# alipbcs/ZetaRay

Hardware: NVIDIA H100
Metric: Mpaths/s (1spp ReSTIR PT, 1080p) (higher is better)
Workload: dtype f32

## Files before the change

zetaray_b200/csrc/rdi.cu:

```cuda
#include "zr_pixel.cuh"
#include "zr_planes.h"
#include "zr_schedule.h"

#include "zr_rdi.cuh"

namespace zr
{
namespace
{
#ifndef ZR_RDI_THREADS
#define ZR_RDI_THREADS 512
#endif
    __global__ void ZR_LB(ZR_RDI_THREADS) k_di_temporal(SceneDev sc, FrameView f, DIParams prm, zr_rdi_reservoir* __restrict__ resCurr,
        const zr_rdi_reservoir* __restrict__ resPrev, uint2* __restrict__ target, float4* __restrict__ finalImg, uint32_t dispX, uint32_t dispY,
        const uint32_t* __restrict__ order)
    {
        const zr_frame_constants& fc = f.fc;
        uint2 sg = make_uint2(0, 0);
        const uint32_t groupFlat = order[blockIdx.x] * (ZR_RDI_THREADS / 64) + (threadIdx.x >> 6);
        const uint32_t tInGroup = threadIdx.x & 63;
        uint2 px = make_uint2(0xffffffffu, 0xffffffffu);
        if (groupFlat < dispX * dispY)
            px = SwizzleThreadGroup(groupFlat, 0, tInGroup & 7, tInGroup >> 3, 8, 8, dispX, 16, 4, 16 * dispY, sg);
        const long long t0 = clock64();
        bool act = !(px.x >= f.W || px.y >= f.H || px.y < prm.rowBegin || px.y >= prm.rowEnd);
        const uint32_t x = px.x, y = px.y;
        const size_t idx = act ? (size_t)y * f.W + x : 0;
        if (act)
        {
            const GFlags flags = FlagsAt(f.core, f.W, x, y);
            if (flags.invalid)
            {
                finalImg[idx] = f4(0, 0, 0, 0);
                act = false;
            }
            else if (flags.emissive && !prm.spatial)
            {
                WriteEmissive(fc, f, finalImg, idx);
                act = false;
            }
        }
        Pixel p;
        p.surface = BSDF::ShadingData::InitEmpty();
        p.pos = f3(0); p.normal = f3(0); p.roughness = 0;
        RNG rng_thread; rng_thread.State = 0;
        int numBsdfSamples = 0;
        if (act)
        {
            p = LoadPixel(f, sc, f.core, f.coat, x, y, false, x, y);
            rng_thread = RNG::Init(x, y, fc.FrameNum);
            numBsdfSamples = (!p.surface.GlossSpecular() && p.roughness < 0.3f) ? 2 : 1;
        }
        RNG rng_group = RNG::Init(groupFlat % dispX, groupFlat / dispX, fc.FrameNum);
        const uint32_t sampleSetIdx = rng_group.UniformUintBounded_Faster(sc.numSampleSets);
        Reservoir r = RIS_InitialCandidates_Sync(act, sc, p.pos, p.normal, p.roughness, p.surface, sampleSetIdx, numBsdfSamples, rng_thread);
        if (prm.temporal)
        {
            float2 motionVec = f2(0, 0);
            TemporalCandidate tc; tc.valid = false; tc.px = tc.py = 0; tc.pos = tc.normal = f3(0);
            tc.surface = BSDF::ShadingData::InitEmpty();
            ZR_PHASE();
            if (act)
            {
                motionVec = unpack_snorm16x2(__ldg(&f.me[idx].x));
                const float2 currUV = f2((float)x + 0.5f, (float)y + 0.5f) / f2((float)f.W, (float)f.H);
                const float2 prevUV = currUV - motionVec;
                tc = FindTemporalCandidate(f, sc, p.pos, p.normal, p.roughness, p.surface, prevUV);
            }
            TemporalResample1_Sync(act && tc.valid, sc, p.pos, p.normal, p.surface, tc, resPrev, f.W, r, rng_thread);
            if (act && prm.spatial)
            {
                const bool disoccluded = !tc.valid && (dot(motionVec, motionVec) > 0);
                r.target = disoccluded ? -r.target : r.target;
                WriteTarget(target, idx, r.target);
                r.target = Math::Sanitize(r.target);
            }
        }
        AccountCost(prm.costMap, f.W, f.H, px.x, px.y, t0);
        if (!act)
            return;
        if (prm.temporal || prm.reset)
        {
            zr_rdi_reservoir rec;
            r.Write(rec, prm.M_max);
            StoreRdi(&resCurr[idx], rec);
        }
        if (!prm.spatial || !prm.temporal)
            WriteFinal(fc, finalImg, idx, r.target * r.W);
    }

    __global__ void ZR_LB(ZR_RDI_THREADS) k_di_spatial(SceneDev sc, FrameView f, DIParams prm, const zr_rdi_reservoir* __restrict__ resCurr,
        const uint2* __restrict__ target, float4* __restrict__ finalImg, uint32_t dispX, uint32_t dispY,
        const uint32_t* __restrict__ order)
    {
        const zr_frame_constants& fc = f.fc;
        uint2 sg = make_uint2(0, 0);
        const uint32_t groupFlat = order[blockIdx.x] * (ZR_RDI_THREADS / 64) + (threadIdx.x >> 6);
        const uint32_t tInGroup = threadIdx.x & 63;
        uint2 px = make_uint2(0xffffffffu, 0xffffffffu);
        if (groupFlat < dispX * dispY)
            px = SwizzleThreadGroup(groupFlat, 0, tInGroup & 7, tInGroup >> 3, 8, 8, dispX, 16, 4, 16 * dispY, sg);
        const long long t0 = clock64();
        bool active = px.x < f.W && px.y < f.H && px.y >= prm.rowBegin && px.y < prm.rowEnd;
        const int x = (int)px.x, y = (int)px.y;
        const size_t idx = active ? (size_t)y * f.W + x : 0;
        if (active)
        {
            const GFlags flags = FlagsAt(f.core, f.W, x, y);
            if (flags.invalid) active = false;
            else if (flags.emissive)
            {
                WriteEmissive(fc, f, finalImg, idx);
                active = false;
            }
        }
        Pixel p;
        p.surface = BSDF::ShadingData::InitEmpty();
        p.pos = f3(0); p.normal = f3(0); p.roughness = 0; p.z = 0;
        Reservoir r = Reservoir::Init();
        bool disoccluded = false;
        if (active)
        {
            p = LoadPixel(f, sc, f.core, f.coat, x, y, false, x, y);
            zr_rdi_reservoir rec;
            LoadRdi(&resCurr[idx], rec);
            r = Reservoir::Load(rec);
            if (r.lightIdx != UINT32_MAX_)
            {
                const zr_emissive_tri& tri = sc.emissives[r.lightIdx];
                r.lightID = tri.ID;
                const float3 vtx0 = Light::Vtx0(tri);
                const float3 vtx1 = Light::DecodeEmissiveTriV1(tri);
                const float3 vtx2 = Light::DecodeEmissiveTriV2(tri);
                r.lightPos = (1.0f - r.bary.x - r.bary.y) * vtx0 + r.bary.x * vtx1 + r.bary.y * vtx2;
                r.lightNormal = cross(vtx1 - vtx0, vtx2 - vtx0);
                r.lightNormal = dot(r.lightNormal, r.lightNormal) == 0 ? r.lightNormal : normalize(r.lightNormal);
                r.doubleSided = Light::IsDoubleSided(tri);
                r.target = LoadTarget(target, idx);
                disoccluded = r.target.x < 0 || r.target.y < 0 || r.target.z < 0;
                r.target = abs3(r.target);
            }
        }
        const uint32_t waveDisoccluded = __popc(__ballot_sync(0xffffffffu, active && disoccluded));
        RNG rng_group = RNG::Init(groupFlat % dispX, groupFlat / dispX, fc.FrameNum);
        rng_group.UniformUintBounded_Faster(sc.numSampleSets);
        const bool extra = !prm.stochasticSpatial || (rng_group.Uniform() < 0.6f);
        if (prm.extraDisocclusion)
            disoccluded = disoccluded && (waveDisoccluded > 3);
        int numSamples = extra ? 2 : 1;
        numSamples = !disoccluded ? numSamples : 4;
        RNG rng = RNG::Init((uint32_t)x, (uint32_t)y, fc.FrameNum);
        const float u0 = rng.Uniform();
        const int offset = (int)rng.UniformUintBounded_Faster(8);
        const float theta = u0 * TWO_PI;
        float sinTheta, cosTheta;
        zr_sincosf(theta, &sinTheta, &cosTheta);
        PairwiseMIS pairwiseMIS = PairwiseMIS::Init((uint32_t)numSamples, r);
        float3 samplePos[4]; int spx[4], spy[4]; uint32_t k = 0;
        ZR_PHASE();
        for (int i = 0; i < 4; i++)
        {
            if (!(active && i < numSamples)) continue;
            const float2 sampleUV = f2(c_disk32[((offset + i) & 31) * 2], c_disk32[((offset + i) & 31) * 2 + 1]);
            float2 rotated;
            rotated.x = dot(sampleUV, f2(cosTheta, -sinTheta));
            rotated.y = dot(sampleUV, f2(sinTheta, cosTheta));
            rotated = rotated * 16.0f;
            const float fx = fmaxf(rintf((float)x + rotated.x), 0.0f), fy = fmaxf(rintf((float)y + rotated.y), 0.0f);
            if (fx >= (float)f.W || fy >= (float)f.H) continue;
            const int qx = (int)fx, qy = (int)fy;
            float rough_i;
            const GFlags flags_i = FlagsAt(f.core, f.W, qx, qy, &rough_i);
            if (flags_i.invalid || flags_i.emissive) continue;
            const Pixel pi = LoadPixel(f, sc, f.core, f.coat, qx, qy, false, qx, qy);
            bool valid = PlaneHeuristicDI(pi.pos, p.normal, p.pos, p.z);
            valid = valid && (fabsf(rough_i - p.roughness) < 0.15f);
            if (!valid) continue;
            samplePos[k] = pi.pos; spx[k] = qx; spy[k] = qy;
            k++;
        }
        pairwiseMIS.k = k;
        for (uint32_t i = 0; i < 4; i++)
        {
            const bool go = active && (i < k);
            if (!__syncthreads_or(go))
                break;
            Pixel pi;
            pi.normal = f3(0);
            BSDF::ShadingData surface_i = BSDF::ShadingData::InitEmpty();
            Reservoir r_spatial = Reservoir::Init();
            float3 pos_i = f3(0);
            if (go)
            {
                pi = LoadPixel(f, sc, f.core, f.coat, spx[i], spy[i], false, spx[i], spy[i]);
                const uint4 c = ld128(&f.core[(size_t)spy[i] * f.W + spx[i]]);
                const float3 bc = f3((float)(c.z & 0xff) / 255.0f, (float)((c.z >> 8) & 0xff) / 255.0f, (float)((c.z >> 16) & 0xff) / 255.0f);
                const float bw = pi.flags.subsurface ? (float)(c.z >> 24) / 255.0f : 0.0f;
                pos_i = samplePos[i];
                const float3 wo_i = normalize(pi.origin - pos_i);
                surface_i = BSDF::ShadingData::Init(pi.normal, wo_i, pi.flags.metallic, pi.roughness, bc, BSDF::ETA_AIR,
                    pi.eta_next, pi.flags.transmissive, 0.0f, to_half(bw), pi.surface.coat_weight, pi.surface.coat_color,
                    pi.coatRoughness, pi.coatIor, sc.rho);
                zr_rdi_reservoir recN;
                LoadRdi(&resCurr[(size_t)spy[i] * f.W + spx[i]], recN);
                r_spatial = Reservoir::Load(recN);
            }
            pairwiseMIS.Stream_Sync(go, sc, r, p.pos, p.normal, p.surface, r_spatial, pos_i, pi.normal, surface_i, rng);
        }
        AccountCost(prm.costMap, f.W, f.H, px.x, px.y, t0);
        if (!active)
            return;
        pairwiseMIS.End(r, rng);
        const Reservoir rs = pairwiseMIS.r_s;
        WriteFinal(fc, finalImg, idx, rs.target * rs.W);
    }
}
}

struct zr_direct_pass
{
    uint32_t width = 0, height = 0;
    struct Sized
    {
        zr::Planes planes{ "zr_direct_pass" };
        zr_rdi_reservoir* d_res[2] = { nullptr, nullptr };
        uint2* d_target = nullptr;
        float4* d_final = nullptr;
    } sz;
    int currTemporalIdx = 0;
    bool isTemporalReservoirValid = false;
    bool resetTemporalTextures = true;
    bool patternLoaded = false;
    zr_direct_params params = Defaults();
    zr::LightingStrip strip{ "zr_direct_pass" };

    static zr_direct_params Defaults()
    {
        zr_direct_params p{};
        p.temporal_resample = 1; p.spatial_resample = 1; p.stochastic_spatial = 1; p.extra_disocclusion_sampling = 1;
        p.M_max = 20; p.alpha_min = 0.05f * 0.05f;
        return p;
    }
    zr_status Setup() { return ZR_OK; }
    zr_status OnWindowResized(uint32_t w, uint32_t h)
    {
        const size_t n = (size_t)w * h;
        Sized next;
        for (int i = 0; i < 2; i++) ZR_TRY(next.planes.Alloc(next.d_res[i], n));
        ZR_TRY(next.planes.Alloc(next.d_target, n));
        ZR_TRY(next.planes.Alloc(next.d_final, n));
        ZR_TRY(next.planes.Clear());
        sz = std::move(next);
        width = w; height = h;
        strip.ForgetSize();
        ResetFlags();
        return ZR_OK;
    }
    void ResetFlags() { currTemporalIdx = 0; isTemporalReservoirValid = false; resetTemporalTextures = true; }
    zr_status ResetTemporal()
    {
        ZR_TRY(sz.planes.Clear());
        ResetFlags();
        return ZR_OK;
    }
    zr_status LoadPattern()
    {
        if (patternLoaded) return ZR_OK;
        float pat[64];
        zr_status st = zr::read_asset("zr_direct_pass", "disk32.bin", pat, sizeof(pat));
        if (st != ZR_OK) return st;
        ZR_CUDA(cudaMemcpyToSymbol(zr::c_disk32, pat, 256));
        patternLoaded = true;
        return ZR_OK;
    }
    zr_status Render(const zr_frame_inputs* in, cudaStream_t stream)
    {
        using namespace zr;
        FrameView f;
        zr_status st = LightingFrame("zr_direct_pass", in, width, height, f);
        if (st != ZR_OK) return st;
        st = LoadPattern();
        if (st != ZR_OK) return st;
        const bool doTemporal = isTemporalReservoirValid && params.temporal_resample;
        const bool doSpatial = doTemporal && params.spatial_resample;
        if (doTemporal && (!in->prev.d_core || !in->prev.d_coat))
        {
            set_error("zr_direct_pass_render: temporal reuse needs the previous G-buffer");
            return ZR_ERR_INVALID_ARG;
        }
        DIParams prm{ doTemporal, doSpatial, params.stochastic_spatial, params.extra_disocclusion_sampling, params.M_max,
            params.alpha_min, resetTemporalTextures, strip.rowBegin, strip.ClampedRowEnd(height), strip.d_costMap };
        const uint32_t dispX = (width + 7) / 8, dispY = (height + 7) / 8;
        const int cur = currTemporalIdx;
        st = strip.Schedule(width, height, 8, 8, ZR_RDI_THREADS / 64);
        if (st != ZR_OK) return st;
        const BlockSchedule& sched = strip.sched;
        ZR_PROF("k_di_temporal", stream);
        k_di_temporal<<<sched.count, ZR_RDI_THREADS, 0, stream>>>(in->scene->dev, f, prm, sz.d_res[cur], sz.d_res[1 - cur], sz.d_target, sz.d_final, dispX, dispY, sched.d_order);
        ZR_LAUNCH_CHECK();
        strip.Exchange(sz.d_res[cur], width, height, 32u, stream);
        if (doSpatial)
        {
            ZR_PROF("k_di_spatial", stream);
            k_di_spatial<<<sched.count, ZR_RDI_THREADS, 0, stream>>>(in->scene->dev, f, prm, sz.d_res[cur], sz.d_target, sz.d_final, dispX, dispY, sched.d_order);
            ZR_LAUNCH_CHECK();
        }
        isTemporalReservoirValid = true;
        currTemporalIdx = 1 - cur;
        resetTemporalTextures = false;
        return ZR_OK;
    }
};

extern "C"
{
    zr_status zr_direct_pass_create(uint32_t width, uint32_t height, zr_direct_pass** out) { return zr::CreatePass("zr_direct_pass", width, height, out); }
    zr_status zr_direct_pass_resize(zr_direct_pass* p, uint32_t width, uint32_t height) { return zr::ResizePass("zr_direct_pass", p, width, height); }
    zr_status zr_direct_pass_reset_temporal(zr_direct_pass* p) { return zr::ResetPass(p); }
    zr_status zr_direct_pass_default_params(zr_direct_params* out) { return zr::DefaultParams<zr_direct_pass>(out); }
    zr_status zr_direct_pass_set_params(zr_direct_pass* p, const zr_direct_params* params)
    {
        if (!p || !params) return ZR_ERR_INVALID_ARG;
        if (params->M_max == 0 || params->M_max > 31) { zr::set_error("zr_direct_pass_set_params: M_max must be in 1..31 (5-bit field)"); return ZR_ERR_INVALID_ARG; }
        p->params = *params;
        return ZR_OK;
    }
    zr_status zr_direct_pass_render(zr_direct_pass* p, const zr_frame_inputs* in, void* stream)
    {
        if (!p) return ZR_ERR_INVALID_ARG;
        return p->Render(in, (cudaStream_t)stream);
    }
    zr_status zr_direct_pass_set_rows(zr_direct_pass* p, uint32_t y0, uint32_t y1) { return p ? p->strip.SetRows(y0, y1, p->height) : ZR_ERR_INVALID_ARG; }
    zr_status zr_direct_pass_set_halo_exchange(zr_direct_pass* p, zr_halo_exchange_fn fn, void* user) { return p ? p->strip.SetHaloExchange(fn, user) : ZR_ERR_INVALID_ARG; }
    zr_status zr_direct_pass_set_schedule_costs(zr_direct_pass* p, const double* h_tile_cost, uint32_t tiles_x, uint32_t tiles_y)
    {
        return p ? p->strip.SetScheduleCosts(h_tile_cost, tiles_x, tiles_y, p->width, p->height) : ZR_ERR_INVALID_ARG;
    }
    zr_status zr_direct_pass_set_cost_map(zr_direct_pass* p, void* d_cycles) { return p ? p->strip.SetCostMap(d_cycles) : ZR_ERR_INVALID_ARG; }
    zr_status zr_direct_pass_get_output(zr_direct_pass* p, zr_direct_output id, zr_image2d* out)
    {
        if (!p || !out) return ZR_ERR_INVALID_ARG;
        const uint32_t w = p->width, h = p->height;
        switch (id)
        {
        case ZR_DIRECT_FINAL: *out = zr_image2d{ p->sz.d_final, w, h, w * 16u, 16u }; break;
        case ZR_DIRECT_RESERVOIR_CURR: *out = zr_image2d{ p->sz.d_res[1 - p->currTemporalIdx], w, h, w * 32u, 32u }; break;
        case ZR_DIRECT_TARGET: *out = zr_image2d{ p->sz.d_target, w, h, w * 8u, 8u }; break;
        default: zr::set_error("zr_direct_pass_get_output: unknown output id"); return ZR_ERR_INVALID_ARG;
        }
        return ZR_OK;
    }
    zr_status zr_direct_pass_describe_io(zr_direct_pass* p, zr_resource_use* uses, int* n)
    {
        if (!p || !uses || !n) return ZR_ERR_INVALID_ARG;
        uses[0] = zr_resource_use{ ZR_RES_GBUFFER_CURR, 0 };
        uses[1] = zr_resource_use{ ZR_RES_GBUFFER_PREV, 0 };
        uses[2] = zr_resource_use{ ZR_RES_SCENE_BVH, 0 };
        uses[3] = zr_resource_use{ ZR_RES_ALIAS_TABLE, 0 };
        uses[4] = zr_resource_use{ ZR_RES_DI_FINAL, 1 };
        *n = 5;
        return ZR_OK;
    }
    void zr_direct_pass_destroy(zr_direct_pass* p) { delete p; }
}
```

zetaray_b200/csrc/zr_rdi.cuh:

```cuda
#pragma once
#include "zr_pixel.cuh"

namespace zr
{
namespace
{
    struct DIParams
    {
        uint32_t temporal, spatial, stochasticSpatial, extraDisocclusion, M_max; float alpha_min; uint32_t reset;
        uint32_t rowBegin, rowEnd;
        unsigned long long* costMap;
    };

    __constant__ float c_disk32[64];

struct Reservoir
{
    float w_sum, W; float3 le; uint32_t lightIdx; float2 bary; uint32_t M;
    float3 target; uint32_t lightID; float3 lightPos, lightNormal; bool doubleSided;

    static ZR_D Reservoir Init()
    {
        Reservoir r;
        r.le = f3(0); r.M = 0; r.w_sum = 0; r.W = 0; r.lightIdx = UINT32_MAX_; r.bary = f2(0, 0);
        r.target = f3(0); r.lightID = UINT32_MAX_; r.lightPos = f3(0); r.lightNormal = f3(0); r.doubleSided = false;
        return r;
    }
    ZR_D bool Update(float weight, float3 le_, uint32_t lightIdx_, float2 bary_, RNG& rng)
    {
        if (weight != weight) return false;
        M += 1;
        if (weight == 0) return false;
        w_sum += weight;
        if (rng.Uniform() < (weight / w_sum))
        {
            le = le_; lightIdx = lightIdx_; bary = bary_;
            return true;
        }
        return false;
    }
    static ZR_D Reservoir Load(const zr_rdi_reservoir& s)
    {
        Reservoir r = Init();
        r.le = f3(half_lo(s.le_rg), half_hi(s.le_rg), half_lo(s.le_b_meta));
        r.M = (s.le_b_meta >> 16) & 0x1f;
        r.w_sum = s.w_sum; r.W = s.W;
        r.lightIdx = s.lightIdx;
        r.bary = Math::DecodeUNorm2(s.bary);
        return r;
    }
    ZR_D void Write(zr_rdi_reservoir& s, uint32_t M_max) const
    {
        uint32_t M_capped = M < M_max ? M : M_max;
        s.bary = Math::EncodeUNorm2(bary);
        s.le_rg = pack_half2(le.x, le.y);
        s.le_b_meta = (uint32_t)zr_f32_to_f16(le.z) | (M_capped << 16);
        s.lightIdx = lightIdx;
        s.w_sum = w_sum; s.W = W;
        s.pad[0] = 0; s.pad[1] = 0;
    }
};

ZR_D void WriteTarget(uint2* target, size_t idx, float3 t)
{
    t = Math::Sanitize(t);
    target[idx] = make_uint2(pack_half2(t.x, t.y), pack_half2(t.z, 0.0f));
}
ZR_D float3 LoadTarget(const uint2* target, size_t idx)
{
    uint2 p = target[idx];
    return f3(half_lo(p.x), half_hi(p.x), half_lo(p.y));
}

struct BSDFHitInfo { uint32_t emissiveTriIdx; float2 bary; float3 lightPos; float t; bool hit; };

ZR_D BSDFHitInfo FindClosestHitDI(const SceneDev& sc, float3 pos, float3 normal, float3 wi, bool transmissive)
{
    BSDFHitInfo ret;
    ret.hit = false; ret.emissiveTriIdx = UINT32_MAX_; ret.bary = f2(0, 0); ret.lightPos = f3(0); ret.t = 0;
    float ndotwi = dot(normal, wi);
    if (ndotwi == 0) return ret;
    bool wiBackface = ndotwi < 0;
    if (wiBackface)
    {
        if (transmissive) normal = -normal;
        else return ret;
    }
    const float3 adjustedOrigin = RTU::OffsetRayRTG(pos, normal);
    RayHit h = TraceClosest(sc, adjustedOrigin, wi, wiBackface ? 3e-4f : 0.0f, FLT_MAX_);
    if (h.hit)
    {
        const uint32_t meshIdx = __ldg(&sc.triMesh[h.tri]);
        const uint32_t baseEmissive = __ldg(&sc.instances[meshIdx].BaseEmissiveTriOffset);
        if (baseEmissive == UINT32_MAX_)
            return ret;
        ret.emissiveTriIdx = baseEmissive + (h.tri - __ldg(&sc.meshFirstTri[meshIdx]));
        ret.bary = h.bary;
        ret.lightPos = mad(h.t, wi, adjustedOrigin);
        ret.t = h.t;
        ret.hit = true;
    }
    return ret;
}

struct EmissiveData
{
    float3 wi; float t; uint32_t ID; float3 lightPos, lightNormal; bool doubleSided;
    static ZR_D EmissiveData Init(const SceneDev& sc, uint32_t lightIdx, float2 bary)
    {
        EmissiveData ret;
        const zr_emissive_tri& tri = sc.emissives[lightIdx];
        ret.ID = tri.ID;
        const float3 vtx0 = Light::Vtx0(tri);
        const float3 vtx1 = Light::DecodeEmissiveTriV1(tri);
        const float3 vtx2 = Light::DecodeEmissiveTriV2(tri);
        ret.lightPos = (1.0f - bary.x - bary.y) * vtx0 + bary.x * vtx1 + bary.y * vtx2;
        ret.lightNormal = cross(vtx1 - vtx0, vtx2 - vtx0);
        ret.lightNormal = dot(ret.lightNormal, ret.lightNormal) == 0 ? ret.lightNormal : normalize(ret.lightNormal);
        ret.doubleSided = Light::IsDoubleSided(tri);
        ret.wi = f3(0); ret.t = 0;
        return ret;
    }
    ZR_D void SetSurfacePos(float3 pos)
    {
        wi = lightPos - pos;
        t = dot(wi, wi) == 0 ? 0 : length(wi);
        wi = t == 0 ? f3(0) : wi / t;
        lightNormal = doubleSided && dot(-wi, lightNormal) < 0 ? -lightNormal : lightNormal;
    }
    ZR_D float dWdA() const
    {
        float cosThetaPrime = saturate(dot(lightNormal, -wi));
        return t == 0 ? 0 : cosThetaPrime / (t * t);
    }
};

#define ZR_PHASE() __syncthreads()
ZR_D Reservoir RIS_InitialCandidates_Sync(bool act, const SceneDev& sc, float3 pos, float3 normal, float roughness, BSDF::ShadingData surface,
    uint32_t sampleSetIdx, int numBsdfSamples, RNG& rng)
{
    Reservoir r = Reservoir::Init();
    const bool specular = surface.GlossSpecular() && (surface.metallic || surface.specTr) && (!surface.Coated() || surface.CoatSpecular());
    const int numLightSamples = !specular ? 3 : 0;
    for (int s_b = 0; s_b < 2; s_b++)
    {
        const bool go = act && (s_b < numBsdfSamples);
        BSDF::BSDFSample bsdfSample = BSDF::BSDFSample::Init();
        ZR_PHASE();
        if (go)
            bsdfSample = BSDF::SampleBSDF_NoDiffuse(normal, surface, rng);
        ZR_PHASE();
        BSDFHitInfo hitInfo;
        hitInfo.hit = false;
        if (go)
            hitInfo = FindClosestHitDI(sc, pos, normal, bsdfSample.wi, surface.Transmissive());
        ZR_PHASE();
        if (go)
        {
            float3 wi = bsdfSample.wi;
            float pdf_w = bsdfSample.pdf;
            float w_b = 0;
            float3 le = f3(0), lightNormal = f3(0), target = f3(0);
            uint32_t emissiveID = UINT32_MAX_;
            bool doubleSided = false;
            if (hitInfo.hit)
            {
                const zr_emissive_tri& emissive = sc.emissives[hitInfo.emissiveTriIdx];
                le = Light::Le_EmissiveTriangle(emissive);
                const float3 vtx0 = Light::Vtx0(emissive);
                const float3 vtx1 = Light::DecodeEmissiveTriV1(emissive);
                const float3 vtx2 = Light::DecodeEmissiveTriV2(emissive);
                lightNormal = cross(vtx1 - vtx0, vtx2 - vtx0);
                float twoArea = length(lightNormal);
                lightNormal = dot(lightNormal, lightNormal) == 0 ? f3(0) : lightNormal / twoArea;
                lightNormal = Light::IsDoubleSided(emissive) && dot(-wi, lightNormal) < 0 ? -lightNormal : lightNormal;
                doubleSided = Light::IsDoubleSided(emissive);
                emissiveID = emissive.ID;
                if (dot(-wi, lightNormal) > 0)
                {
                    const float lightSourcePdf = sc.aliasTable[hitInfo.emissiveTriIdx].CachedP_Orig;
                    const float pdf_light = lightSourcePdf * (1.0f / (0.5f * twoArea));
                    const float dwdA = saturate(dot(lightNormal, -wi)) / (hitInfo.t * hitInfo.t);
                    pdf_w *= dwdA;
                    const bool sampleIsSpecular = (surface.GlossSpecular() && bsdfSample.lobe == BSDF::GLOSSY_R) ||
                        (surface.CoatSpecular() && bsdfSample.lobe == BSDF::COAT);
                    float denom = (float)numBsdfSamples * pdf_w + (!sampleIsSpecular ? 1.0f : 0.0f) * (float)numLightSamples * pdf_light;
                    const float m_i = 1.0f / denom;
                    target = le * bsdfSample.f * dwdA;
                    w_b = m_i * Math::Luminance(target);
                }
            }
            if (r.Update(w_b, le, hitInfo.emissiveTriIdx, hitInfo.bary, rng))
            {
                r.target = target; r.lightID = emissiveID; r.lightPos = hitInfo.lightPos; r.lightNormal = lightNormal; r.doubleSided = doubleSided;
            }
        }
    }
    for (int s_l = 0; s_l < 3; s_l++)
    {
        const bool go = act && (s_l < numLightSamples);
        Light::LightSample lightSample;
        float3 le = f3(0), target = f3(0), wi = f3(0);
        float pdf_light = 0, t = 0, dwdA = 0;
        uint32_t emissiveIdx = 0, lightID = UINT32_MAX_;
        bool doubleSided = false, facing = false;
        ZR_PHASE();
        if (go)
        {
            lightSample = Light::SampleLight(sc, pos, sampleSetIdx, rng, false);
            le = lightSample.le;
            pdf_light = lightSample.pdf;
            emissiveIdx = lightSample.idx;
            lightID = lightSample.ID;
            doubleSided = lightSample.twoSided;
            wi = lightSample.pos - pos;
            const bool isZero = dot(wi, wi) == 0;
            t = isZero ? 0 : length(wi);
            wi = isZero ? wi : wi / t;
            dwdA = isZero ? 0 : saturate(dot(lightSample.normal, -wi)) / (t * t);
            surface.SetWi(wi, normal);
            facing = dot(lightSample.normal, -wi) > 0;
            if (facing)
                target = le * BSDF::Unified(surface).f * dwdA;
        }
        ZR_PHASE();
        if (go && facing && (dot(target, target) > 0))
            target *= Visibility_Segment(sc, pos, wi, t, normal, lightID, surface.Transmissive()) ? 1.0f : 0.0f;
        ZR_PHASE();
        if (go)
        {
            const float denom = (float)numLightSamples * pdf_light + (float)numBsdfSamples * BSDF::BSDFSamplerPdf_NoDiffuse(normal, surface, wi) * dwdA;
            const float m_l = denom > 0 ? 1.0f / denom : 0;
            const float w_l = m_l * Math::Luminance(target);
            if (r.Update(w_l, le, emissiveIdx, lightSample.bary, rng))
            {
                r.target = target; r.lightID = lightID; r.lightNormal = lightSample.normal; r.lightPos = lightSample.pos; r.doubleSided = doubleSided;
            }
        }
    }
    float targetLum = Math::Luminance(r.target);
    r.W = targetLum > 0.0f ? r.w_sum / targetLum : 0.0f;
    return r;
}

ZR_D bool PlaneHeuristicDI(float3 samplePos, float3 currNormal, float3 currPos, float linearDepth, float tolerance = 1e-1f)
{
    float planeDist = dot(currNormal, samplePos - currPos);
    return fabsf(planeDist) <= tolerance * linearDepth;
}

struct TemporalCandidate { BSDF::ShadingData surface; float3 pos, normal; int px, py; bool valid; };

ZR_D TemporalCandidate FindTemporalCandidate(const FrameView& f, const SceneDev& sc, float3 pos, float3 normal, float roughness, const BSDF::ShadingData& surface, float2 prevUV)
{
    TemporalCandidate c; c.valid = false; c.px = c.py = 0; c.pos = c.normal = f3(0);
    if (prevUV.x < 0.0f || prevUV.y < 0.0f || prevUV.x > 1.0f || prevUV.y > 1.0f) return c;
    const float2 renderDim = f2((float)f.W, (float)f.H);
    float2 pp = prevUV * renderDim;
    int ppx = (int)pp.x, ppy = (int)pp.y;
    float prevRoughness;
    GFlags prevFlags = FlagsAt(f.pcore, f.W, ppx, ppy, &prevRoughness);
    if (prevFlags.invalid || prevFlags.emissive || (fabsf(prevRoughness - roughness) > 0.15f) ||
        (prevFlags.metallic != surface.metallic) || (prevFlags.transmissive != surface.specTr))
        return c;
    Pixel p = LoadPixel(f, sc, f.pcore, f.pcoat, ppx, ppy, true, ppx, ppy);
    if (!PlaneHeuristicDI(p.pos, normal, pos, p.z))
        return c;
    c.surface = p.surface; c.px = ppx; c.py = ppy; c.pos = p.pos; c.normal = p.normal; c.valid = true;
    return c;
}

ZR_D void TemporalResample1_Sync(bool act, const SceneDev& sc, float3 pos, float3 normal, const BSDF::ShadingData& surface, TemporalCandidate candidate,
    const zr_rdi_reservoir* prevRes, uint32_t W, Reservoir& r_curr, RNG& rng)
{
    Reservoir r_prev = Reservoir::Init();
    if (act)
        r_prev = Reservoir::Load(prevRes[(size_t)candidate.py * W + candidate.px]);
    const uint32_t newM = r_curr.M + r_prev.M;
    const bool doCtT = act && (r_curr.w_sum != 0);
    float3 wi_offset = f3(0);
    float t_offset = 0, targetLum_offset = 0;
    float3 target_offset = f3(0);
    if (doCtT)
    {
        wi_offset = r_curr.lightPos - candidate.pos;
        const bool isZero = dot(wi_offset, wi_offset) == 0;
        t_offset = isZero ? 0 : length(wi_offset);
        wi_offset = isZero ? wi_offset : wi_offset / t_offset;
        candidate.surface.SetWi(wi_offset, candidate.normal);
        float3 lightNormal = r_curr.lightNormal;
        if (r_curr.doubleSided && dot(-wi_offset, lightNormal) < 0)
            lightNormal = -lightNormal;
        float cosThetaPrime = saturate(dot(lightNormal, -wi_offset));
        const float dwdA = isZero ? 0 : cosThetaPrime / (t_offset * t_offset);
        target_offset = r_curr.le * dwdA;
    }
    ZR_PHASE();
    if (doCtT)
    {
        target_offset *= BSDF::Unified(candidate.surface).f;
        targetLum_offset = Math::Luminance(target_offset);
    }
    ZR_PHASE();
    if (doCtT)
    {
        if (targetLum_offset > 0)
            targetLum_offset *= Visibility_Segment(sc, candidate.pos, wi_offset, t_offset, candidate.normal, r_curr.lightID,
                candidate.surface.Transmissive()) ? 1.0f : 0.0f;
        const float numerator = (float)r_curr.M * Math::Luminance(r_curr.target);
        const float denom = numerator + (float)r_prev.M * targetLum_offset * 1.0f;
        const float m_curr = denom > 0 ? numerator / denom : 0;
        r_curr.w_sum *= m_curr;
    }
    const bool doTtC = act && (r_prev.lightIdx != UINT32_MAX_);
    EmissiveData prevEmissive;
    BSDF::ShadingData surfaceWi = surface;
    float3 target_curr = f3(0);
    if (doTtC)
    {
        prevEmissive = EmissiveData::Init(sc, r_prev.lightIdx, r_prev.bary);
        prevEmissive.SetSurfacePos(pos);
        const float dwdA = prevEmissive.dWdA();
        surfaceWi.SetWi(prevEmissive.wi, normal);
        target_curr = r_prev.le * dwdA;
    }
    ZR_PHASE();
    if (doTtC)
        target_curr *= BSDF::Unified(surfaceWi).f;
    ZR_PHASE();
    if (doTtC)
    {
        if (dot(target_curr, target_curr) > 0)
            target_curr *= Visibility_Segment(sc, pos, prevEmissive.wi, prevEmissive.t, normal, prevEmissive.ID, surfaceWi.Transmissive()) ? 1.0f : 0.0f;
        const float targetLum_curr = Math::Luminance(target_curr);
        if (targetLum_curr > 0)
        {
            const float targetLum_prev = r_prev.W > 0 ? r_prev.w_sum / r_prev.W : 0;
            const float numerator = (float)r_prev.M * targetLum_prev;
            const float denom = numerator / 1.0f + (float)r_curr.M * targetLum_curr;
            const float m_prev = denom > 0 ? numerator / denom : 0;
            const float w_prev = m_prev * targetLum_curr * r_prev.W;
            if (r_curr.Update(w_prev, r_prev.le, r_prev.lightIdx, r_prev.bary, rng))
                r_curr.target = target_curr;
        }
    }
    if (act)
    {
        float targetLum = Math::Luminance(r_curr.target);
        r_curr.W = targetLum > 0.0f ? r_curr.w_sum / targetLum : 0.0f;
        r_curr.M = newM;
    }
}

struct PairwiseMIS
{
    Reservoir r_s; float m_c; float M_s; uint32_t k;
    static ZR_D PairwiseMIS Init(uint32_t numStrategies, const Reservoir& r_c)
    {
        PairwiseMIS ret;
        ret.r_s = Reservoir::Init(); ret.m_c = 1.0f; ret.M_s = to_half((float)r_c.M); ret.k = numStrategies;
        return ret;
    }
    ZR_D float Compute_m_i(const Reservoir& r_c, const Reservoir& r_i, float targetLum, float jacobian) const
    {
        const float p_i_y_i = r_i.W > 0 ? r_i.w_sum / r_i.W : 0;
        const float p_c_y_i = targetLum;
        float numerator = (float)r_i.M * p_i_y_i;
        float denom = (numerator / jacobian) + ((float)r_c.M / (float)k) * p_c_y_i;
        return denom > 0 ? numerator / denom : 0;
    }
    ZR_D void Update_m_c(const Reservoir& r_c, const Reservoir& r_i, float targetLum, float jacobian)
    {
        const float p_i_y_c = targetLum;
        const float p_c_y_c = Math::Luminance(r_c.target);
        const float numerator = (float)r_i.M * p_i_y_c * jacobian;
        const float denom = numerator + ((float)r_c.M / (float)k) * p_c_y_c;
        m_c += 1 - (numerator / denom);
    }
    ZR_D void Stream_Sync(bool act, const SceneDev& sc, const Reservoir& r_c, float3 pos_c, float3 normal_c, BSDF::ShadingData surface_c, const Reservoir& r_i,
        float3 pos_i, float3 normal_i, BSDF::ShadingData surface_i, RNG& rng)
    {
        float3 target_c_y_i = f3(0), target_i_y_c = f3(0.0f);
        float m_i = 0;
        const bool has_i = act && (r_i.lightIdx != UINT32_MAX_);
        const float jacobian_i_to_c = 1;
        EmissiveData emissive_i;
        if (has_i)
        {
            emissive_i = EmissiveData::Init(sc, r_i.lightIdx, r_i.bary);
            emissive_i.SetSurfacePos(pos_c);
            float dwdA = emissive_i.dWdA();
            surface_c.SetWi(emissive_i.wi, normal_c);
            target_c_y_i = r_i.le * dwdA;
        }
        ZR_PHASE();
        if (has_i && (dot(target_c_y_i, target_c_y_i) > 0))
            target_c_y_i *= Visibility_Segment(sc, pos_c, emissive_i.wi, emissive_i.t, normal_c, emissive_i.ID, surface_c.Transmissive()) ? 1.0f : 0.0f;
        ZR_PHASE();
        if (has_i)
        {
            target_c_y_i *= BSDF::Unified(surface_c).f;
            const float targetLum = Math::Luminance(target_c_y_i);
            m_i = Compute_m_i(r_c, r_i, targetLum, jacobian_i_to_c);
        }
        float jacobian_c_to_i = 0;
        const bool has_c = act && (r_c.lightIdx != UINT32_MAX_);
        float3 wi_i = f3(0);
        float t_i = 0;
        if (has_c)
        {
            jacobian_c_to_i = 1;
            wi_i = r_c.lightPos - pos_i;
            const bool isZero = dot(wi_i, wi_i) == 0;
            t_i = isZero ? 0 : length(wi_i);
            wi_i = isZero ? f3(0) : wi_i / t_i;
            surface_i.SetWi(wi_i, normal_i);
            const float3 lightNormal = dot(r_c.lightNormal, -wi_i) < 0 && r_c.doubleSided ? -r_c.lightNormal : r_c.lightNormal;
            const float cosThetaPrime = saturate(dot(lightNormal, -wi_i));
            const float dwdA = isZero ? 0 : cosThetaPrime / (t_i * t_i);
            target_i_y_c = r_c.le * dwdA;
        }
        ZR_PHASE();
        if (has_c && (dot(target_i_y_c, target_i_y_c) > 0))
            target_i_y_c *= Visibility_Segment(sc, pos_i, wi_i, t_i, normal_i, r_c.lightID, surface_i.Transmissive()) ? 1.0f : 0.0f;
        ZR_PHASE();
        if (has_c)
            target_i_y_c *= BSDF::Unified(surface_i).f;
        if (act)
        {
            const float targetLum = Math::Luminance(target_i_y_c);
            Update_m_c(r_c, r_i, targetLum, jacobian_c_to_i);
            if (r_i.lightIdx != UINT32_MAX_)
            {
                const float w_i = m_i * Math::Luminance(target_c_y_i) * r_i.W;
                if (r_s.Update(w_i, r_i.le, r_i.lightIdx, r_i.bary, rng))
                    r_s.target = target_c_y_i;
            }
            M_s = to_half(M_s + (float)r_i.M);
        }
    }
    ZR_D void End(const Reservoir& r_c, RNG& rng)
    {
        const float w_c = m_c * r_c.w_sum;
        if (r_s.Update(w_c, r_c.le, r_c.lightIdx, r_c.bary, rng))
            r_s.target = r_c.target;
        r_s.M = (uint32_t)M_s;
        const float targetLum = Math::Luminance(r_s.target);
        r_s.W = targetLum > 0 ? r_s.w_sum / (targetLum * (1 + (float)k)) : 0;
    }
};


    ZR_D void LoadRdi(const zr_rdi_reservoir* __restrict__ p, zr_rdi_reservoir& r)
    {
        const uint4* q = reinterpret_cast<const uint4*>(p);
        uint4 v[2] = { q[0], q[1] };
        memcpy(&r, v, 32);
    }
    ZR_D void StoreRdi(zr_rdi_reservoir* __restrict__ p, const zr_rdi_reservoir& r)
    {
        uint4 v[2];
        memcpy(v, &r, 32);
        uint4* q = reinterpret_cast<uint4*>(p);
        q[0] = v[0]; q[1] = v[1];
    }

    ZR_D void WriteFinal(const zr_frame_constants& fc, float4* __restrict__ finalImg, size_t idx, float3 li)
    {
        li = isnan3(li) ? f3(0) : li;
        if (fc.Accumulate && fc.CameraStatic && fc.NumFramesCameraStatic > 1)
        {
            const float4 prev = finalImg[idx];
            finalImg[idx] = f4(prev.x + li.x, prev.y + li.y, prev.z + li.z, prev.w);
        }
        else
            finalImg[idx] = f4(li.x, li.y, li.z, 0.0f);
    }

    ZR_D void WriteEmissive(const zr_frame_constants& fc, const FrameView& f, float4* __restrict__ finalImg, size_t idx)
    {
        const float3 le = unpack_r11g11b10(__ldg(&f.me[idx].y));
        if (fc.Accumulate && fc.CameraStatic)
        {
            const float4 prev = finalImg[idx];
            finalImg[idx] = f4(prev.x + le.x, prev.y + le.y, prev.z + le.z, prev.w);
        }
        else
            finalImg[idx] = f4(le.x, le.y, le.z, 0.0f);
    }
}
}
```

zetaray_b200/csrc/zr_rt.cuh:

```cuda
#pragma once
#include "zr_scene.cuh"
#include "zr_bsdf.cuh"

namespace zr
{
constexpr uint32_t UINT32_MAX_ = 0xffffffffu;

namespace RTU
{
    ZR_D float3 OffsetRayRTG(float3 pos, float3 geometricNormal)
    {
        const float origin = 1.0f / 32.0f;
        const float float_scale = 1.0f / 65536.0f;
        const float int_scale = 256.0f;
        int ofx = (int)(int_scale * geometricNormal.x), ofy = (int)(int_scale * geometricNormal.y), ofz = (int)(int_scale * geometricNormal.z);
        auto adj = [](float p, int of) { return asfloat((uint32_t)((int)asuint(p) + ((p < 0) ? -of : of))); };
        float3 p_i = f3(adj(pos.x, ofx), adj(pos.y, ofy), adj(pos.z, ofz));
        return f3(fabsf(pos.x) < origin ? pos.x + float_scale * geometricNormal.x : p_i.x,
                  fabsf(pos.y) < origin ? pos.y + float_scale * geometricNormal.y : p_i.y,
                  fabsf(pos.z) < origin ? pos.z + float_scale * geometricNormal.z : p_i.z);
    }
}

constexpr float T_MIN_REFL_RAY = 1e-6f;
constexpr float T_MIN_TR_RAY = 5e-5f;

struct Hit
{
    bool hit; float t; float2 uv; float3 normal; uint32_t ID; uint32_t meshIdx; uint32_t matIdx;
};

struct HitEmissive
{
    bool hit; float t; uint32_t geoIdx, primIdx, emissiveTriIdx; float2 bary; float3 lightPos;
    ZR_D bool HitWasEmissive() const { return emissiveTriIdx != UINT32_MAX_; }
};

ZR_D Hit HitAttributes(const SceneDev& sc, uint32_t meshIdx, uint32_t primIdx, float2 bary, float t)
{
    Hit ret;
    const zr_mesh_instance meshData = LoadInstance(sc, meshIdx);
    ret.hit = true;
    ret.t = t;
    ret.matIdx = meshData.MatIdx;
    ret.meshIdx = meshIdx;
    uint32_t tri = primIdx * 3 + meshData.BaseIdxOffset;
    const VertexD V0 = LoadVertex(sc, __ldg(&sc.indices[tri]) + meshData.BaseVtxOffset);
    const VertexD V1 = LoadVertex(sc, __ldg(&sc.indices[tri + 1]) + meshData.BaseVtxOffset);
    const VertexD V2 = LoadVertex(sc, __ldg(&sc.indices[tri + 2]) + meshData.BaseVtxOffset);
    float4 q = normalize(Math::DecodeNormalized4(meshData.Rotation));
    float3 s = h3(meshData.Scale);
    float tmp = 1 - bary.x - bary.y;
    float2 uv = f2(mad(bary.y, V2.uv.x, tmp * V0.uv.x), mad(bary.y, V2.uv.y, tmp * V0.uv.y));
    uv = f2(mad(bary.x, V1.uv.x, uv.x), mad(bary.x, V1.uv.y, uv.y));
    ret.uv = uv;
    float3 v0_n = Math::DecodeOct32(V0.normal);
    float3 v1_n = Math::DecodeOct32(V1.normal);
    float3 v2_n = Math::DecodeOct32(V2.normal);
    float3 hitNormal = mad(bary.y, v2_n, tmp * v0_n);
    hitNormal = mad(bary.x, v1_n, hitNormal);
    const float3 scaleInv = 1.0f / s;
    hitNormal *= scaleInv;
    hitNormal = Math::RotateVector(hitNormal, q);
    hitNormal = normalize(hitNormal);
    ret.normal = hitNormal;
    ret.ID = RNG::PCG3d(make_uint3(meshIdx, 0u, primIdx)).x;
    return ret;
}

ZR_D HitEmissive FindClosestEmissive(const SceneDev& sc, float3 pos, float3 normal, float3 wi, bool transmissive)
{
    HitEmissive ret;
    ret.hit = false;
    ret.emissiveTriIdx = UINT32_MAX_;
    ret.t = 0; ret.geoIdx = 0; ret.primIdx = 0; ret.bary = f2(0, 0); ret.lightPos = f3(0);
    bool wiBackface = dot(normal, wi) <= 0;
    if (wiBackface)
    {
        if (transmissive) normal = -normal;
        else return ret;
    }
    const float3 adjustedOrigin = RTU::OffsetRayRTG(pos, normal);
    RayHit h = TraceClosest(sc, adjustedOrigin, wi, wiBackface ? T_MIN_TR_RAY : T_MIN_REFL_RAY, FLT_MAX_);
    if (h.hit)
    {
        ret.hit = true;
        ret.bary = h.bary;
        ret.t = h.t;
        ret.geoIdx = __ldg(&sc.triMesh[h.tri]);
        ret.primIdx = h.tri - __ldg(&sc.meshFirstTri[ret.geoIdx]);
        const uint32_t baseEmissive = __ldg(&sc.instances[ret.geoIdx].BaseEmissiveTriOffset);
        if (baseEmissive == UINT32_MAX_)
            return ret;
        ret.emissiveTriIdx = baseEmissive + ret.primIdx;
        ret.lightPos = mad(h.t, wi, adjustedOrigin);
    }
    return ret;
}

ZR_D Hit FindClosest(const SceneDev& sc, float3 pos, float3 normal, float3 wi, bool transmissive)
{
    Hit ret;
    ret.hit = false;
    ret.ID = UINT32_MAX_;
    ret.t = 0; ret.uv = f2(0, 0); ret.normal = f3(0); ret.meshIdx = 0; ret.matIdx = 0;
    float ndotwi = dot(normal, wi);
    if (ndotwi == 0)
        return ret;
    bool wiBackface = ndotwi < 0;
    if (wiBackface)
    {
        if (!transmissive) return ret;
        normal = -normal;
    }
    const float3 adjustedOrigin = RTU::OffsetRayRTG(pos, normal);
    RayHit h = TraceClosest(sc, adjustedOrigin, wi, wiBackface ? T_MIN_TR_RAY : T_MIN_REFL_RAY, FLT_MAX_);
    if (h.hit)
        {
        const uint32_t mesh = __ldg(&sc.triMesh[h.tri]);
        ret = HitAttributes(sc, mesh, h.tri - __ldg(&sc.meshFirstTri[mesh]), h.bary, h.t);
    }
    return ret;
}

ZR_D bool Visibility_Segment(const SceneDev& sc, float3 origin, float3 wi, float rayT, float3 normal, uint32_t triID,
    bool transmissive)
{
    if (triID == UINT32_MAX_) return false;
    if (rayT < 1e-6f) return false;
    float ndotwi = dot(normal, wi);
    if (ndotwi == 0) return false;
    bool wiBackface = ndotwi < 0;
    if (wiBackface)
    {
        if (transmissive) normal = -normal;
        else return false;
    }
    const float3 adjustedOrigin = RTU::OffsetRayRTG(origin, normal);
    const float tMin = 3e-6f;
    const float tMax = Math::PrevFloat32(rayT * 0.999f - Math::NextFloat32(tMin));
    return !TraceAnyExcept(sc, adjustedOrigin, wi, tMin, tMax, triID);
}

ZR_D bool Visibility_Segment_Precise(const SceneDev& sc, float3 origin, float3 wi, float rayT, float3 normal, uint32_t triID,
    bool transmissive)
{
    if (triID == UINT32_MAX_) return false;
    if (rayT < 1e-6f) return false;
    float ndotwi = dot(normal, wi);
    if (ndotwi == 0) return false;
    bool wiBackface = ndotwi < 0;
    if (wiBackface)
    {
        if (transmissive) normal = -normal;
        else return false;
    }
    const float3 adjustedOrigin = RTU::OffsetRayRTG(origin, normal);
    const RayHit h = TraceClosest(sc, adjustedOrigin, wi, 3e-6f, rayT);
    if (h.hit)
        return triID == TriID(sc, h.tri);
    return true;
}

ZR_D bool GetMaterialData(const SceneDev& sc, float3 wo, float eta_curr, Hit& hitInfo, BSDF::ShadingData& surface, float& eta)
{
    const zr_material mat = LoadMaterial(sc, hitInfo.matIdx);
    const bool hitBackface = dot(wo, hitInfo.normal) < 0;
    eta = BSDF::DEFAULT_ETA_MAT;
    if (!Mat::DoubleSided(mat) && hitBackface)
        return false;
    if (Mat::DoubleSided(mat) && hitBackface)
        hitInfo.normal = -hitInfo.normal;
    float3 baseColor = Mat::GetBaseColorFactor(mat);
    float metallic = Mat::Metallic(mat) ? 1.0f : 0.0f;
    float roughness = Mat::GetSpecularRoughness(mat);
    bool tr = Mat::Transmissive(mat);
    eta = Mat::GetSpecularIOR(mat);
    float trDepth = tr ? Mat::GetTransmissionDepth(mat) : 0;
    float eta_next = eta_curr == BSDF::ETA_AIR ? eta : BSDF::ETA_AIR;
    float subsurface = Mat::ThinWalled(mat) ? to_half(Mat::GetSubsurface(mat)) : 0;
    float coat_weight = Mat::GetCoatWeight(mat);
    float3 coat_color = Mat::GetCoatColor(mat);
    float coat_roughness = Mat::GetCoatRoughness(mat);
    float coat_ior = Mat::GetCoatIOR(mat);
    surface = BSDF::ShadingData::Init(hitInfo.normal, wo, metallic >= 0.9f, roughness, baseColor, eta_curr, eta_next, tr,
        trDepth, subsurface, coat_weight, coat_color, coat_roughness, coat_ior, sc.rho);
    return true;
}

namespace Light
{
    enum TYPE : uint32_t { NONE = 0, SUN = 1, SKY = 2, EMISSIVE = 3 };
    ZR_D TYPE TypeFromValue(uint32_t x) { return x <= 2 ? (TYPE)x : EMISSIVE; }

    ZR_D float3 DecodeEmissiveTriV1(const zr_emissive_tri& tri)
    {
        float2 v = f2((float)tri.V0V1[0] / 65535.0f, (float)tri.V0V1[1] / 65535.0f);
        float3 decoded = Math::DecodeUnitVector(v);
        return mad(decoded, zr_f16_to_f32(tri.EdgeLengths[0]), f3(tri.Vtx0[0], tri.Vtx0[1], tri.Vtx0[2]));
    }
    ZR_D float3 DecodeEmissiveTriV2(const zr_emissive_tri& tri)
    {
        float2 v = f2((float)tri.V0V2[0] / 65535.0f, (float)tri.V0V2[1] / 65535.0f);
        float3 decoded = Math::DecodeUnitVector(v);
        return mad(decoded, zr_f16_to_f32(tri.EdgeLengths[1]), f3(tri.Vtx0[0], tri.Vtx0[1], tri.Vtx0[2]));
    }
    ZR_D bool IsDoubleSided(const zr_emissive_tri& tri) { return tri.PackedA & (1u << 25); }
    ZR_D float3 Vtx0(const zr_emissive_tri& tri) { return f3(tri.Vtx0[0], tri.Vtx0[1], tri.Vtx0[2]); }

    ZR_D float3 Le_EmissiveTriangle(const zr_emissive_tri& tri)
    {
        const float3 emissiveFactor = Math::UnpackRGB8(tri.PackedA);
        const float emissiveStrength = zr_f16_to_f32((uint16_t)(tri.PackedB >> 16));
        float3 le = emissiveFactor * emissiveStrength;
        if (Math::Luminance(le) == 0)
            return f3(0.0f);
        return le;
    }

    struct AliasTableSample { uint32_t idx; float pdf; };
    ZR_D AliasTableSample SampleAlias(const zr_alias_entry* table, uint32_t numEmissiveTriangles, RNG& rng)
    {
        AliasTableSample ret;
        uint32_t u0 = rng.UniformUintBounded(numEmissiveTriangles);
        const uint4 raw = __ldg(reinterpret_cast<const uint4*>(table + u0));
        zr_alias_entry s; s.CachedP_Orig = asfloat(raw.x); s.CachedP_Alias = asfloat(raw.y); s.P_Curr = asfloat(raw.z); s.Alias = raw.w;
        if (rng.Uniform() < s.P_Curr) { ret.pdf = s.CachedP_Orig; ret.idx = u0; return ret; }
        ret.pdf = s.CachedP_Alias;
        ret.idx = s.Alias;
        return ret;
    }

    struct LightSample { float3 pos, normal, le; float2 bary; float pdf; uint32_t idx, ID; bool twoSided; };
    struct EmissiveTriSample { float3 pos, normal; float2 bary; float pdf; };
    ZR_D EmissiveTriSample SampleEmissiveTri(float3 pos, const zr_emissive_tri& tri, RNG& rng, bool reverseNormalIfTwoSided = true)
    {
        EmissiveTriSample ret;
        float2 u = rng.Uniform2D();
        ret.bary = Sampling::UniformSampleTriangle(u);
        const float3 vtx0 = Vtx0(tri);
        const float3 vtx1 = DecodeEmissiveTriV1(tri);
        const float3 vtx2 = DecodeEmissiveTriV2(tri);
        ret.pos = (1.0f - ret.bary.x - ret.bary.y) * vtx0 + ret.bary.x * vtx1 + ret.bary.y * vtx2;
        ret.normal = cross(vtx1 - vtx0, vtx2 - vtx0);
        bool normalIs0 = dot(ret.normal, ret.normal) == 0;
        float twoArea = length(ret.normal);
        ret.pdf = normalIs0 ? 0.0f : 2.0f / twoArea;
        ret.normal = normalIs0 ? ret.normal : ret.normal / twoArea;
        ret.normal = reverseNormalIfTwoSided && IsDoubleSided(tri) && dot(pos - ret.pos, ret.normal) < 0 ? -ret.normal : ret.normal;
        return ret;
    }

    ZR_D LightSample SampleLight(const SceneDev& sc, float3 pos, uint32_t sampleSetIdx, RNG& rng, bool advanceRng)
    {
        LightSample ls;
        if (sc.sampleSetSize > 0)
        {
            const uint32_t u = rng.UniformUintBounded_Faster(sc.sampleSetSize);
            const zr_presampled_tri* p = sc.sampleSets + (size_t)sampleSetIdx * sc.sampleSetSize + u;
            const uint2* q = reinterpret_cast<const uint2*>(p);
            const uint2 q0 = __ldg(q), q1 = __ldg(q + 1), q2 = __ldg(q + 2), q3 = __ldg(q + 3), c = __ldg(q + 4);
            const uint4 a = make_uint4(q0.x, q0.y, q1.x, q1.y);
            const uint4 b = make_uint4(q2.x, q2.y, q3.x, q3.y);
            ls.pos = f3(asfloat(a.x), asfloat(a.y), asfloat(a.z));
            ls.normal = Math::DecodeOct32(a.w);
            ls.bary = Math::DecodeUNorm2(b.w);
            ls.le = f3(zr_f16_to_f32((uint16_t)(c.x & 0xffff)), zr_f16_to_f32((uint16_t)(c.x >> 16)), zr_f16_to_f32((uint16_t)(c.y & 0xffff)));
            ls.pdf = asfloat(b.x); ls.ID = b.y; ls.idx = b.z;
            ls.twoSided = (c.y >> 16) != 0;
            if (ls.twoSided && dot(pos - ls.pos, ls.normal) < 0)
                ls.normal = -ls.normal;
            if (advanceRng)
                rng.Uniform3D();
        }
        else
        {
            AliasTableSample entry = SampleAlias(sc.aliasTable, sc.numEmissives, rng);
            const zr_emissive_tri& tri = sc.emissives[entry.idx];
            const EmissiveTriSample ts = SampleEmissiveTri(pos, tri, rng);
            ls.pos = ts.pos; ls.normal = ts.normal; ls.bary = ts.bary;
            ls.le = Le_EmissiveTriangle(tri);
            ls.pdf = entry.pdf * ts.pdf; ls.idx = entry.idx; ls.ID = tri.ID; ls.twoSided = IsDoubleSided(tri);
        }
        return ls;
    }
}
namespace LVG
{
    ZR_D uint32_t FlattenVoxelIndex(uint32_t x, uint32_t y, uint32_t z, uint32_t dx, uint32_t dy) { return z * dx * dy + y * dx + x; }

    ZR_D float3 VoxelCenter(int vx, int vy, int vz, int dx, int dy, int dz, float3 voxelExtents, const float viewInv[3][4], float offset_y)
    {
        const int hx = dx >> 1, hy = dy >> 1, hz = dz >> 1;
        int cx = vx - hx, cy = vy - hy, cz = vz - hz;
        cx += vx < hx ? 1 : 0; cy += vy < hy ? 1 : 0; cz += vz < hz ? 1 : 0;
        cy *= -1;
        const float3 corner = f3((float)(cx * 2), (float)(cy * 2), (float)(cz * 2)) * voxelExtents;
        const float3 s = f3(Math::SignNotZero((float)cx), Math::SignNotZero((float)cy), Math::SignNotZero((float)cz));
        float3 centerV = corner + voxelExtents * s;
        centerV.y += offset_y;
        return Math::mul3x4(viewInv, centerV);
    }

    ZR_D bool MapPosToVoxel(float3 pos, int dx, int dy, int dz, float3 voxelExtents, const float view[3][4], int& ox, int& oy, int& oz, float offset_y)
    {
        float3 posV = Math::mul3x4(view, pos);
        posV.y -= offset_y;
        const int hx = dx >> 1, hy = dy >> 1, hz = dz >> 1;
        float3 voxel = f3(floorf(fabsf(posV.x) / (2 * voxelExtents.x)), floorf(fabsf(posV.y) / (2 * voxelExtents.y)), floorf(fabsf(posV.z) / (2 * voxelExtents.z)));
        if (voxel.x >= (float)hx || voxel.y >= (float)hy || voxel.z >= (float)hz)
            return false;
        voxel = voxel * f3(Math::SignNotZero(posV.x), Math::SignNotZero(posV.y), Math::SignNotZero(posV.z));
        voxel.y *= -1;
        ox = (int)voxel.x + hx - (posV.x < 0 ? 1 : 0);
        oy = (int)voxel.y + hy - (posV.y >= 0 ? 1 : 0);
        oz = (int)voxel.z + hz - (posV.z < 0 ? 1 : 0);
        return true;
    }
}

namespace LVG
{
    struct VoxelLight { float3 pos, normal, le; float pdf; uint32_t ID; bool twoSided; };
    ZR_D bool Sample(const SceneDev& sc, float3 pos, float3 voxelExtents, float offset_y, const float view[3][4], VoxelLight& out, RNG& rng)
    {
        const float3 u = rng.Uniform3D();
        const float3 posJittered = pos + (u * 2.0f - 1.0f) * voxelExtents;
        int vx, vy, vz;
        if (!MapPosToVoxel(posJittered, (int)sc.lvgDim[0], (int)sc.lvgDim[1], (int)sc.lvgDim[2], voxelExtents, view, vx, vy, vz, offset_y))
            return false;
        const uint32_t start = FlattenVoxelIndex((uint32_t)vx, (uint32_t)vy, (uint32_t)vz, sc.lvgDim[0], sc.lvgDim[1]) * 64u;
        const uint32_t k = rng.UniformUintBounded_Faster(64u);
        const uint4* q = reinterpret_cast<const uint4*>(sc.lvg + start + k);
        const uint4 a = __ldg(q), b = __ldg(q + 1);
        out.pos = f3(asfloat(a.x), asfloat(a.y), asfloat(a.z));
        out.normal = Math::DecodeOct32(a.w);
        out.pdf = asfloat(b.x); out.ID = b.y;
        out.le = f3(zr_f16_to_f32((uint16_t)(b.z & 0xffff)), zr_f16_to_f32((uint16_t)(b.z >> 16)), zr_f16_to_f32((uint16_t)(b.w & 0xffff)));
        out.twoSided = (b.w >> 16) != 0;
        return true;
    }
}
}
```

Measured before the change: 287.8.

## Batch both spatial-reuse shadow rays into one phase via shared-memory staging

```diff
diff --git a/zetaray_b200/csrc/rdi.cu b/zetaray_b200/csrc/rdi.cu
--- a/zetaray_b200/csrc/rdi.cu
+++ b/zetaray_b200/csrc/rdi.cu
@@ -8,9 +8,6 @@
 {
 namespace
 {
-#ifndef ZR_RDI_THREADS
-#define ZR_RDI_THREADS 512
-#endif
     __global__ void ZR_LB(ZR_RDI_THREADS) k_di_temporal(SceneDev sc, FrameView f, DIParams prm, zr_rdi_reservoir* __restrict__ resCurr,
         const zr_rdi_reservoir* __restrict__ resPrev, uint2* __restrict__ target, float4* __restrict__ finalImg, uint32_t dispX, uint32_t dispY,
         const uint32_t* __restrict__ order)
diff --git a/zetaray_b200/csrc/zr_rdi.cuh b/zetaray_b200/csrc/zr_rdi.cuh
--- a/zetaray_b200/csrc/zr_rdi.cuh
+++ b/zetaray_b200/csrc/zr_rdi.cuh
@@ -136,6 +136,9 @@
 };
 
 #define ZR_PHASE() __syncthreads()
+#ifndef ZR_RDI_THREADS
+#define ZR_RDI_THREADS 512
+#endif
 ZR_D Reservoir RIS_InitialCandidates_Sync(bool act, const SceneDev& sc, float3 pos, float3 normal, float roughness, BSDF::ShadingData surface,
     uint32_t sampleSetIdx, int numBsdfSamples, RNG& rng)
 {
@@ -390,18 +393,7 @@
             emissive_i = EmissiveData::Init(sc, r_i.lightIdx, r_i.bary);
             emissive_i.SetSurfacePos(pos_c);
             float dwdA = emissive_i.dWdA();
-            surface_c.SetWi(emissive_i.wi, normal_c);
             target_c_y_i = r_i.le * dwdA;
-        }
-        ZR_PHASE();
-        if (has_i && (dot(target_c_y_i, target_c_y_i) > 0))
-            target_c_y_i *= Visibility_Segment(sc, pos_c, emissive_i.wi, emissive_i.t, normal_c, emissive_i.ID, surface_c.Transmissive()) ? 1.0f : 0.0f;
-        ZR_PHASE();
-        if (has_i)
-        {
-            target_c_y_i *= BSDF::Unified(surface_c).f;
-            const float targetLum = Math::Luminance(target_c_y_i);
-            m_i = Compute_m_i(r_c, r_i, targetLum, jacobian_i_to_c);
         }
         float jacobian_c_to_i = 0;
         const bool has_c = act && (r_c.lightIdx != UINT32_MAX_);
@@ -414,18 +406,37 @@
             const bool isZero = dot(wi_i, wi_i) == 0;
             t_i = isZero ? 0 : length(wi_i);
             wi_i = isZero ? f3(0) : wi_i / t_i;
-            surface_i.SetWi(wi_i, normal_i);
             const float3 lightNormal = dot(r_c.lightNormal, -wi_i) < 0 && r_c.doubleSided ? -r_c.lightNormal : r_c.lightNormal;
             const float cosThetaPrime = saturate(dot(lightNormal, -wi_i));
             const float dwdA = isZero ? 0 : cosThetaPrime / (t_i * t_i);
             target_i_y_c = r_c.le * dwdA;
         }
         ZR_PHASE();
-        if (has_c && (dot(target_i_y_c, target_i_y_c) > 0))
-            target_i_y_c *= Visibility_Segment(sc, pos_i, wi_i, t_i, normal_i, r_c.lightID, surface_i.Transmissive()) ? 1.0f : 0.0f;
-        ZR_PHASE();
+        const bool trace_i = has_i && (dot(target_c_y_i, target_c_y_i) > 0), trace_c = has_c && (dot(target_i_y_c, target_i_y_c) > 0);
+        ShadowSegment seg_c_y_i = DeadShadowSegment(), seg_i_y_c = DeadShadowSegment();
+        if (trace_i)
+            seg_c_y_i = SetupShadowSegment(pos_c, emissive_i.wi, emissive_i.t, normal_c, emissive_i.ID, surface_c.Transmissive());
+        if (trace_c)
+            seg_i_y_c = SetupShadowSegment(pos_i, wi_i, t_i, normal_i, r_c.lightID, surface_i.Transmissive());
+        bool visible_c_y_i, visible_i_y_c;
+        TraceShadowSegmentPair<ZR_RDI_THREADS>(sc, seg_c_y_i, seg_i_y_c, visible_c_y_i, visible_i_y_c);
+        if (trace_i)
+            target_c_y_i *= visible_c_y_i ? 1.0f : 0.0f;
+        if (trace_c)
+            target_i_y_c *= visible_i_y_c ? 1.0f : 0.0f;
+        ZR_PHASE();
+        if (has_i)
+        {
+            surface_c.SetWi(emissive_i.wi, normal_c);
+            target_c_y_i *= BSDF::Unified(surface_c).f;
+            const float targetLum = Math::Luminance(target_c_y_i);
+            m_i = Compute_m_i(r_c, r_i, targetLum, jacobian_i_to_c);
+        }
         if (has_c)
+        {
+            surface_i.SetWi(wi_i, normal_i);
             target_i_y_c *= BSDF::Unified(surface_i).f;
+        }
         if (act)
         {
             const float targetLum = Math::Luminance(target_i_y_c);
diff --git a/zetaray_b200/csrc/zr_rt.cuh b/zetaray_b200/csrc/zr_rt.cuh
--- a/zetaray_b200/csrc/zr_rt.cuh
+++ b/zetaray_b200/csrc/zr_rt.cuh
@@ -123,6 +123,38 @@
     return ret;
 }
 
+constexpr float T_MIN_SHADOW_SEGMENT = 3e-6f;
+struct ShadowSegment { float3 o, d; float tMax; uint32_t ignoreID; bool live; };
+
+ZR_D ShadowSegment DeadShadowSegment()
+{
+    ShadowSegment s; s.o = f3(0); s.d = f3(0); s.tMax = 0; s.ignoreID = UINT32_MAX_; s.live = false;
+    return s;
+}
+ZR_D ShadowSegment SetupShadowSegment(float3 origin, float3 wi, float rayT, float3 normal, uint32_t triID, bool transmissive)
+{
+    ShadowSegment s = DeadShadowSegment();
+    if (triID == UINT32_MAX_) return s;
+    if (rayT < 1e-6f) return s;
+    float ndotwi = dot(normal, wi);
+    if (ndotwi == 0) return s;
+    bool wiBackface = ndotwi < 0;
+    if (wiBackface)
+    {
+        if (transmissive) normal = -normal;
+        else return s;
+    }
+    s.o = RTU::OffsetRayRTG(origin, normal);
+    s.d = wi;
+    s.tMax = Math::PrevFloat32(rayT * 0.999f - Math::NextFloat32(T_MIN_SHADOW_SEGMENT));
+    s.ignoreID = triID;
+    s.live = true;
+    return s;
+}
+ZR_D bool TraceShadowSegment(const SceneDev& sc, const ShadowSegment& s)
+{
+    return s.live && !TraceAnyExcept(sc, s.o, s.d, T_MIN_SHADOW_SEGMENT, s.tMax, s.ignoreID);
+}
 ZR_D bool Visibility_Segment(const SceneDev& sc, float3 origin, float3 wi, float rayT, float3 normal, uint32_t triID,
     bool transmissive)
 {
@@ -140,6 +172,26 @@
     const float tMin = 3e-6f;
     const float tMax = Math::PrevFloat32(rayT * 0.999f - Math::NextFloat32(tMin));
     return !TraceAnyExcept(sc, adjustedOrigin, wi, tMin, tMax, triID);
+}
+template<int THREADS>
+ZR_D void TraceShadowSegmentPair(const SceneDev& sc, const ShadowSegment& s0, const ShadowSegment& s1, bool& visible0, bool& visible1)
+{
+    __shared__ float4 staged[2][2][THREADS];
+    const uint32_t t = threadIdx.x;
+    staged[0][0][t] = make_float4(s0.o.x, s0.o.y, s0.o.z, s0.tMax);
+    staged[0][1][t] = make_float4(s0.d.x, s0.d.y, s0.d.z, asfloat(s0.live ? s0.ignoreID : UINT32_MAX_));
+    staged[1][0][t] = make_float4(s1.o.x, s1.o.y, s1.o.z, s1.tMax);
+    staged[1][1][t] = make_float4(s1.d.x, s1.d.y, s1.d.z, asfloat(s1.live ? s1.ignoreID : UINT32_MAX_));
+    visible0 = false; visible1 = false;
+#pragma unroll 1
+    for (int trip = 0; trip < 2; trip++)
+    {
+        const float4 a = staged[trip][0][t], b = staged[trip][1][t];
+        ShadowSegment s;
+        s.o = f3(a.x, a.y, a.z); s.tMax = a.w; s.d = f3(b.x, b.y, b.z); s.ignoreID = asuint(b.w); s.live = s.ignoreID != UINT32_MAX_;
+        const bool v = TraceShadowSegment(sc, s);
+        if (trip) visible1 = v; else visible0 = v;
+    }
 }
 
 ZR_D bool Visibility_Segment_Precise(const SceneDev& sc, float3 origin, float3 wi, float rayT, float3 normal, uint32_t triID,
```

After: 286.7, median of 6. No clear change (-0.4%).
